# Jabruson/FDN-TIP2025

Measured on AMD Instinct MI355X. Metric: images/sec, FDN (LPNet->FDN forward) 1280x720 bs=8 fp32, higher is better.
Workload: dtype f32

## Files before the change

fdn-tip2025_amd/csrc/fft2d.hip:

```cpp
#include <math.h>

#include "common.hpp"
#include "fft_regs.hpp"

namespace {

constexpr int MAX_STAGES = FDN_FFT_MAX_STAGES;
constexpr int NT = 256;

struct Plan {
    int N;
    int nst;
    int radix[MAX_STAGES];
    const float2* tw;
    int tab_mul;
};

struct Rader {
    int p;
    const int* perm_in;
    const int* perm_out;
    const float2* bhat;
    Plan sub;
};
// ... 408 lines not shown
        float2* out2 = reinterpret_cast<float2*>(out + row0 * W);
        const int live = nrow * M;
        if (M % 2 == 0 && ((reinterpret_cast<uintptr_t>(out) | reinterpret_cast<uintptr_t>(res)) & 15) == 0) {
            const float4* res4 = reinterpret_cast<const float4*>(res2);
            float4* out4 = reinterpret_cast<float4*>(out2);
            const float4* Z4 = reinterpret_cast<const float4*>(Z);
            const int live4 = live / 2;
            for (int base = threadIdx.x; base < live4; base += NT * 4) {
                float4 r[4];
                if (res4) {
#pragma unroll
                    for (int u = 0; u < 4; ++u) r[u] = res4[min(base + NT * u, live4 - 1)];
                }
#pragma unroll
                for (int u = 0; u < 4; ++u) {
                    const int idx = base + NT * u;
                    if (idx >= live4) continue;
                    float4 v = Z4[idx];
                    v.x *= scale; v.y *= scale; v.z *= scale; v.w *= scale;
                    if (res4) {
                        v.x = fmaf(alpha, r[u].x, v.x); v.y = fmaf(alpha, r[u].y, v.y);
                        v.z = fmaf(alpha, r[u].z, v.z); v.w = fmaf(alpha, r[u].w, v.w);
                    }
                    out4[idx] = v;
                }
            }
        } else
        for (int base = threadIdx.x; base < live; base += NT * US) {
            float2 r[US];
            if (res2) {
#pragma unroll
                for (int u = 0; u < US; ++u) r[u] = res2[min(base + NT * u, live - 1)];
            }
#pragma unroll
            for (int u = 0; u < US; ++u) {
                const int idx = base + NT * u;
                if (idx >= live) continue;
                float2 v = Z[idx];
                v.x *= scale;
                v.y *= scale;
                if (res2) {
                    v.x = fmaf(alpha, r[u].x, v.x);
                    v.y = fmaf(alpha, r[u].y, v.y);
                }
                out2[idx] = v;
            }
        }
    }
}

struct ColArgs {
    float2* z;
    int H, Wf, C;
    int tc, tcs;
    long planes;
    const float4* guide;
    const float* wxa;
    const float* wxp;
    float* out_abs;
    float* out_ang;
    int rd_before;
    int fix_real;
    const float* in_mag;
    const float* in_pha;
    int Hin, Wfin;
};

enum { COL_FCAFFN = 0, COL_FWD = 1, COL_INV_POLAR = 2 };

template <int MODE, int BIG, bool INPL>
__global__ __launch_bounds__(NT, (INPL ? 2 : 1)) void fft_cols_kernel(ColArgs a, const Plan p) {
    extern __shared__ __attribute__((aligned(16))) unsigned char smem[];
    const int H = a.H, Wf = a.Wf, tc = a.tc;
    float2* A = reinterpret_cast<float2*>(smem);
    float2* Bf = A + (long)H * tc;
    float2* twl = INPL ? Bf : Bf + (long)H * tc;
    for (int i = threadIdx.x; i < H; i += NT) twl[i] = p.tw[i];
    int plane, col0;
    {
        const int ntile = (Wf + tc - 1) / tc;
        const long total = (long)ntile * a.planes, per_xcd = (total + 7) / 8;
        const long w = (long)(blockIdx.x & 7) * per_xcd + (blockIdx.x >> 3);
        if (w >= total) return;
        const int C = a.C;
        const long grp = w / C;
        const int ch = (int)(w - grp * C);
        plane = (int)(grp / ntile) * C + ch;
        col0 = (int)(grp % ntile) * tc;
    }
    const int ncol = min(tc, Wf - col0);
    float2* zp = a.z + (long)plane * H * Wf;

    const int per = H * tc, tcs = a.tcs, tcm = tc - 1;
    if (MODE == COL_INV_POLAR) {
        constexpr int U = 4;
        for (int base = threadIdx.x; base < per; base += NT * U) {
            float mg[U], ph[U];
#pragma unroll
            for (int u = 0; u < U; ++u) {
                const int idx = base + NT * u, h = idx >> tcs, c = idx & tcm;
                mg[u] = 0.f; ph[u] = 0.f;
                if (idx < per && c < ncol) {
                    const long o = ((long)plane * a.Hin + h) * a.Wfin + col0 + c;
                    mg[u] = a.in_mag[o];
                    ph[u] = a.in_pha[o];
                }
// ... 74 lines not shown
                    float sn, cs;
                    fdn_sincos(ph, &sn, &cs);
                    const float2 v = Z[idx];
                    const float2 r = make_float2(rd1(v.x), rd1(v.y));
                    Z[idx] = cmul(r, make_float2(A_ * cs, -A_ * sn));
                }
            }
        }
    }
    float2* Y = Z;
    if (INPL) fft_run_inplace<true, BIG>(Z, p, twl, tc);
    else Y = fft_run<true, BIG>(Z, other, p, twl, tc, 1, tc, true);
#pragma unroll 8
    for (int idx = threadIdx.x; idx < per; idx += NT) {
        const int h = idx >> tcs, c = idx & tcm;
        if (c < ncol) zp[(long)h * Wf + col0 + c] = Y[idx];
    }
}

using fftr::f2;
using fftr::sfor;

__device__ __forceinline__ rsrc_t cols_rsrc(const void* base, long bytes) {
    return mk_rsrc(base, (unsigned)(bytes > 0x7FFFFFFFL ? 0x7FFFFFFFL : bytes));
}

template <typename K>
int set_lds(K kernel, size_t bytes) {
    if (bytes > 48 * 1024 && !fdn_allow_dynamic_lds(reinterpret_cast<const void*>(kernel), bytes)) return FDN_ERR_LAUNCH;
    return FDN_OK;
}

template <int R, int P> struct ColPlan {
    static constexpr int NJ = R * 8, NT = NJ > 256 ? 320 : 256, KS = 256 + 4;
    static constexpr size_t lds = ((size_t)R * KS + (size_t)(P - 1) * R) * sizeof(float2);
};

template <int R, int P, int MODE>
__global__ __launch_bounds__((ColPlan<R, P>::NT), (3 * ColPlan<R, P>::lds <= 160 * 1024) ? 3 : 2) void fft_cols_rp_kernel(ColArgs a, const float2* __restrict__ twT) {
    constexpr int H = R * P, TC = 256 / P, CJ = 32 / P, NG = 8, KS = ColPlan<R, P>::KS, NJ = R * NG, NT = ColPlan<R, P>::NT;
    static_assert(TC / CJ == NG, "8 column groups");
    extern __shared__ __attribute__((aligned(16))) unsigned char smem_cols[];
    f2* Y = reinterpret_cast<f2*>(smem_cols);
    f2* twl = Y + R * KS;
    const int tid = threadIdx.x, Wf = a.Wf;
    const bool io = NT == 256 || tid < 256;
    for (int i = tid; i < (P - 1) * R; i += NT) twl[i] = f2{twT[R + i].x, twT[R + i].y};
    int plane, col0;
    {
        const int ntile = (Wf + TC - 1) / TC;
        const long total = (long)ntile * a.planes, per_xcd = (total + 7) / 8;
        const long w = (long)(blockIdx.x & 7) * per_xcd + (blockIdx.x >> 3);
        if (w >= total) return;
        const int C = a.C, CH = (C % 8 == 0) ? 8 : 1;
        const long grp = w / CH;
        const int ci = (int)(w - grp * CH);
        const long rest = grp / ntile;
        col0 = (int)(grp - rest * ntile) * TC;
        const int nchunk = C / CH;
        const long b = rest / nchunk;
        plane = (int)(b * C + (rest - b * nchunk) * CH + ci);
    }
    const int c = tid & (TC - 1), n2 = (tid & 255) / TC;
    const bool live = col0 + c < Wf;
    const int col = live ? col0 + c : Wf - 1;
    const long plane_bins = (long)H * Wf;
    const __amdgpu_buffer_rsrc_t rz = cols_rsrc(a.z + (long)plane * plane_bins, plane_bins * 8);
    const unsigned zoff = (unsigned)(n2 * Wf + col) * 8u, zstep = (unsigned)(P * Wf) * 8u;

    if (MODE != COL_INV_POLAR && io) {
        f2 u[R];
        sfor<0, R>([&](auto n1) { u[decltype(n1)::value] = bload2(rz, zoff, (unsigned)decltype(n1)::value * zstep); });
        fftr::dft_nat<R, false>(u);
        sfor<0, R>([&](auto k1) { Y[decltype(k1)::value * KS + tid] = u[decltype(k1)::value]; });
    }

    int jt = tid + 64 * (int)((blockIdx.x >> 3) % (NT / 64));
    if (jt >= NT) jt -= NT;
    const bool worker = jt < NJ;
    const int k1 = worker ? jt >> 3 : 0, cg = jt & 7;
    unsigned binq[CJ];
    bool liveq[CJ];
#pragma unroll
    for (int cc = 0; cc < CJ; ++cc) {
        liveq[cc] = col0 + cc * NG + cg < Wf;
        binq[cc] = (unsigned)(k1 * Wf + (liveq[cc] ? col0 + cc * NG + cg : Wf - 1));
    }
    const unsigned kstep = (unsigned)(R * Wf);
    constexpr int NB = (3 * ColPlan<R, P>::lds <= 160 * 1024) ? 16 : 4, BS = 32 / NB;
    fdn_u32x4 g0[2][BS];
    fdn_u32x2 g1[2][BS];
    __amdgpu_buffer_rsrc_t rg = rz;
    float wa0 = 0, wa1 = 0, wa2 = 0, wp0 = 0, wp1 = 0, wp2 = 0;
    auto gload = [&](auto bb) __attribute__((always_inline)) {
        constexpr int Bb = decltype(bb)::value;
        sfor<0, BS>([&](auto i) {
            constexpr int q = Bb * BS + decltype(i)::value, cc = q / P, k2 = fftr::brev(q % P, P);
            g0[Bb & 1][decltype(i)::value] = __builtin_amdgcn_raw_buffer_load_b128(rg, binq[cc] * 32u, (unsigned)k2 * kstep * 32u, 0);
            g1[Bb & 1][decltype(i)::value] = __builtin_amdgcn_raw_buffer_load_b64(rg, binq[cc] * 32u, (unsigned)k2 * kstep * 32u + 16u, 0);
        });
    };
    if (MODE == COL_FCAFFN) {
        const int b = plane / a.C, ch = plane - b * a.C;
        wa0 = a.wxa[ch * 3]; wa1 = a.wxa[ch * 3 + 1]; wa2 = a.wxa[ch * 3 + 2];
        wp0 = a.wxp[ch * 3]; wp1 = a.wxp[ch * 3 + 1]; wp2 = a.wxp[ch * 3 + 2];
        rg = cols_rsrc(a.guide + (long)b * plane_bins * 2, plane_bins * 32);
        if (worker) gload(std::integral_constant<int, 0>{});
// ... 88 lines not shown
            for (int cc = 0; cc < CJ; ++cc) inq[cc] = (unsigned)(k1 * a.Wfin + ((int)binq[cc] - k1 * Wf)) * 4u;
            const unsigned instep = (unsigned)(R * a.Wfin) * 4u;
            sfor<0, NB>([&](auto bb) {
                constexpr int Bb = decltype(bb)::value;
                float mg[BS], ph[BS];
                sfor<0, BS>([&](auto i) {
                    constexpr int I = decltype(i)::value, q = Bb * BS + I, cc = q / P, k2 = fftr::brev(q % P, P);
                    mg[I] = __uint_as_float(__builtin_amdgcn_raw_buffer_load_b32(rm, inq[cc], (unsigned)k2 * instep, 0));
                    ph[I] = __uint_as_float(__builtin_amdgcn_raw_buffer_load_b32(rp, inq[cc], (unsigned)k2 * instep, 0));
                });
                sfor<0, BS>([&](auto i) {
                    constexpr int I = decltype(i)::value, q = Bb * BS + I;
                    float sn, cs;
                    fdn_sincos(ph[I], &sn, &cs);
                    v[q] = f2{mg[I] * cs, mg[I] * sn};
                });
            });
        }
#pragma unroll
        for (int cc = 0; cc < CJ; ++cc) fftr::fft_dit<P, true>(v + cc * P);
        asm volatile("" ::: "memory");
        sfor<0, P>([&](auto n) {
            constexpr int N2 = decltype(n)::value;
            if constexpr (N2 > 0) {
                const f2 w = twl[(N2 - 1) * R + k1];
#pragma unroll
                for (int cc = 0; cc < CJ; ++cc) v[cc * P + N2] = fftr::cmulc(v[cc * P + N2], w);
            }
#pragma unroll
            for (int cc = 0; cc < CJ; ++cc) yb[N2 * TC + cc * NG] = v[cc * P + N2];
        });
    } else if (MODE == COL_FWD) {
        return;
    }
    __syncthreads();
    if (io) {
        f2 u[R];
        sfor<0, R>([&](auto k) { u[decltype(k)::value] = Y[decltype(k)::value * KS + tid]; });
        fftr::dft_nat<R, true>(u);
        if (live) sfor<0, R>([&](auto n1) { bstore2(u[decltype(n1)::value], rz, zoff, (unsigned)decltype(n1)::value * zstep); });
    }
}

constexpr int row_plan_groups(int R1, int P) {
    int ng = 8;
    while (ng > 1 && (R1 * ng > 256 || ((long)ng * (32 / P) * R1 * (P + 1) + (P - 1) * R1 + R1 * P + 1) * 8 > 80 * 1024)) --ng;
    return ng;
}
template <int R1, int P>
struct RowPlan {
    static constexpr int NG = row_plan_groups(R1, P);
    static constexpr int M = R1 * P, W = 2 * M, Wf = M + 1, CJ = 32 / P, RW = NG * CJ, PS = P + 1, RS = R1 * PS, NJ = R1 * NG;
    static constexpr int NTW = (P - 1) * R1 + Wf;
    static constexpr size_t lds = ((size_t)RW * RS + NTW) * sizeof(float2);
    static_assert(RW * P <= 256 && NJ <= 256 && CJ * P <= 32, "first stage: one thread per (row, n2); second stage: one per (row group, k1) with 32 values");
};

struct RowLN {
    const float* stats;
    const float* gamma;
    const float* beta;
    int C, H;
};

template <int R1, int P, bool LN = false>
__global__ __launch_bounds__(256, 2) void rfft_rows_rp_kernel(const float* __restrict__ in, float2* __restrict__ out, long R,
                                                              const float2* __restrict__ tab, RowLN lnp, int pitch) {
    typedef RowPlan<R1, P> L;
    constexpr int M = L::M, W = L::W, Wf = L::Wf, RW = L::RW, CJ = L::CJ, PS = L::PS, RS = L::RS, NJ = L::NJ;
    extern __shared__ __attribute__((aligned(16))) unsigned char smem[];
    f2* Y = reinterpret_cast<f2*>(smem);
    f2* tw2 = Y + RW * RS;
    f2* tws = tw2 + (P - 1) * R1;
    const int tid = threadIdx.x;
    for (int i = tid; i < L::NTW; i += 256) tw2[i] = f2{tab[i].x, tab[i].y};
    const long row0 = (long)blockIdx.x * RW;
    const int nrow = (int)min((long)RW, R - row0);
    {
        const int n2 = tid & (P - 1), rw = tid / P < RW ? tid / P : RW - 1;
        const int rwc = rw < nrow ? rw : nrow - 1;
        const __amdgpu_buffer_rsrc_t rin = cols_rsrc(in + row0 * W, (long)nrow * W * 4);
        const unsigned voff = (unsigned)(rwc * W + 2 * n2) * 4u;
        f2 u[R1];
        sfor<0, R1>([&](auto n1) { u[decltype(n1)::value] = bload2(rin, voff, (unsigned)(decltype(n1)::value * P * 8)); });
        if constexpr (LN) {
            const long row = row0 + rwc, plane = row / lnp.H;
            const int h = (int)(row - plane * lnp.H), c = (int)(plane % lnp.C);
            const long b = plane / lnp.C, HW = (long)lnp.H * W;
            const __amdgpu_buffer_rsrc_t rs_ = cols_rsrc(lnp.stats, (R / ((long)lnp.C * lnp.H)) * 2 * HW * 4);
            const unsigned so = (unsigned)(b * 2 * HW + h * W + 2 * n2) * 4u;
            const float ga = lnp.gamma[c], be = lnp.beta[c];
            f2 mu[R1], rs[R1];
            sfor<0, R1>([&](auto n1) {
                constexpr int N1 = decltype(n1)::value;
                mu[N1] = bload2(rs_, so, (unsigned)(N1 * P * 8));
                rs[N1] = bload2(rs_, so + (unsigned)HW * 4u, (unsigned)(N1 * P * 8));
            });
            sfor<0, R1>([&](auto n1) {
                constexpr int N1 = decltype(n1)::value;
                u[N1] = (u[N1] - mu[N1]) * rs[N1] * ga + be;
            });
        }
        fftr::dft_nat<R1, false>(u);
        sfor<0, R1>([&](auto k1) { Y[rw * RS + decltype(k1)::value * PS + n2] = u[decltype(k1)::value]; });
    }
    __syncthreads();
    const int jt = (tid + 64 * (int)(blockIdx.x & 3)) & 255;
    const bool worker = jt < NJ;
    const int rg = jt / R1, k1 = jt - rg * R1;
    f2 v[32];
    if (worker) {
        const f2* yb = Y + rg * CJ * RS + k1 * PS;
        sfor<0, P>([&](auto n) {
            constexpr int N2 = decltype(n)::value;
#pragma unroll
            for (int cc = 0; cc < CJ; ++cc) v[cc * P + N2] = yb[cc * RS + N2];
            if constexpr (N2 > 0) {
                const f2 w = tw2[(N2 - 1) * R1 + k1];
#pragma unroll
                for (int cc = 0; cc < CJ; ++cc) v[cc * P + N2] = fftr::cmul(v[cc * P + N2], w);
            }
        });
#pragma unroll
        for (int cc = 0; cc < CJ; ++cc) fftr::dft_nat<P, false>(v + cc * P);
    }
    __syncthreads();
    if (worker) {
        f2* zb = Y + rg * CJ * RS + k1;
        sfor<0, P>([&](auto k2) {
#pragma unroll
            for (int cc = 0; cc < CJ; ++cc) zb[cc * RS + R1 * decltype(k2)::value] = v[cc * P + decltype(k2)::value];
        });
    }
    __syncthreads();
    f2* out2 = reinterpret_cast<f2*>(out) + row0 * pitch;
    const int live = nrow * pitch;
    const float r_Wf = 1.0f / (float)pitch;
#pragma unroll 4
    for (int idx = tid; idx < live; idx += 256) {
        const int s = fdiv(idx, r_Wf), k = idx - s * pitch;
        if (k >= Wf) { out2[idx] = f2{0.f, 0.f}; continue; }
        const f2 zk = Y[s * RS + (k == M ? 0 : k)];
        const f2 zc = Y[s * RS + (k == 0 ? 0 : M - k)];
        const f2 e = 0.5f * f2{zk.x + zc.x, zk.y - zc.y};
        const f2 d = 0.5f * f2{zk.x - zc.x, zk.y + zc.y};
        const f2 o = fftr::mul_ni(d);
        f2 x;
        if (k == 0) x = f2{e.x + o.x, 0.0f};
        else if (k == M) x = f2{e.x - o.x, 0.0f};
        else x = e + fftr::cmul(o, tws[k]);
        out2[idx] = x;
    }
}

template <int R1, int P>
__global__ __launch_bounds__(256, 2) void irfft_rows_rp_kernel(const float2* __restrict__ in, long in_ws, long in_plane_stride,
                                                               float* __restrict__ out, int H, long R, float scale,
                                                               const float* __restrict__ res, float alpha,
                                                               const float2* __restrict__ tab) {
    typedef RowPlan<R1, P> L;
    constexpr int M = L::M, W = L::W, RW = L::RW, CJ = L::CJ, PS = L::PS, RS = L::RS, NJ = L::NJ;
    extern __shared__ __attribute__((aligned(16))) unsigned char smem[];
    f2* Y = reinterpret_cast<f2*>(smem);
    f2* tw2 = Y + RW * RS;
    f2* tws = tw2 + (P - 1) * R1;
    __shared__ long rowoff[RW];
    const int tid = threadIdx.x;
    for (int i = tid; i < L::NTW; i += 256) tw2[i] = f2{tab[i].x, tab[i].y};
    const long row0 = (long)blockIdx.x * RW;
    const int nrow = (int)min((long)RW, R - row0);
    if (tid < RW) {
        const long row = row0 + min(tid, nrow - 1);
        const long plane = row / H, h = row - plane * H;
        rowoff[tid] = plane * in_plane_stride + h * in_ws;
    }
    __syncthreads();
    {
        constexpr int UL = 4, NP = M / 2 + 1, TOT = RW * NP;
        const f2* in2 = reinterpret_cast<const f2*>(in);
        const float r_NP = 1.0f / (float)NP;
        for (int base = tid; base < TOT; base += 256 * UL) {
            f2 xks[UL], xcs[UL];
#pragma unroll
            for (int u = 0; u < UL; ++u) {
                const int idx = min(base + 256 * u, TOT - 1), s = fdiv(idx, r_NP), k = idx - s * NP;
                const f2* src = in2 + rowoff[s];
                xks[u] = src[k];
                xcs[u] = src[M - k];
            }
#pragma unroll
            for (int u = 0; u < UL; ++u) {
                const int idx = base + 256 * u;
                if (idx >= TOT) continue;
                const int s = fdiv(idx, r_NP), k = idx - s * NP;
                f2 xk = xks[u], xc = xcs[u];
                if (k == 0) { xk.y = 0.f; xc.y = 0.f; }
                const f2 e = 0.5f * f2{xk.x + xc.x, xk.y - xc.y};
                const f2 d = 0.5f * f2{xk.x - xc.x, xk.y + xc.y};
                const f2 io = fftr::mul_pi(fftr::cmulc(d, tws[k]));
                f2* row = Y + s * RS;
                row[k] = e + io;
                if (k != 0) {
                    const f2 c = e - io;
                    row[M - k] = f2{c.x, -c.y};
// ... 8 lines not shown
    f2 v[32];
    if (worker) {
        const f2* zb = Y + rg * CJ * RS + k1;
        sfor<0, P>([&](auto k2) {
#pragma unroll
            for (int cc = 0; cc < CJ; ++cc) v[cc * P + decltype(k2)::value] = zb[cc * RS + R1 * decltype(k2)::value];
        });
#pragma unroll
        for (int cc = 0; cc < CJ; ++cc) fftr::dft_nat<P, true>(v + cc * P);
    }
    __syncthreads();
    if (worker) {
        f2* yb = Y + rg * CJ * RS + k1 * PS;
        sfor<0, P>([&](auto n) {
            constexpr int N2 = decltype(n)::value;
            if constexpr (N2 > 0) {
                const f2 w = tw2[(N2 - 1) * R1 + k1];
#pragma unroll
                for (int cc = 0; cc < CJ; ++cc) v[cc * P + N2] = fftr::cmulc(v[cc * P + N2], w);
            }
#pragma unroll
            for (int cc = 0; cc < CJ; ++cc) yb[cc * RS + N2] = v[cc * P + N2];
        });
    }
    __syncthreads();
    {
        const int n2 = tid & (P - 1), rw = tid / P;
        const int rwl = rw < RW ? rw : RW - 1;
        f2 u[R1];
        sfor<0, R1>([&](auto k) { u[decltype(k)::value] = Y[rwl * RS + decltype(k)::value * PS + n2]; });
        fftr::dft_nat<R1, true>(u);
        if (rw < nrow) {
            const __amdgpu_buffer_rsrc_t ro = cols_rsrc(out + row0 * W, (long)nrow * W * 4);
            const __amdgpu_buffer_rsrc_t rr = cols_rsrc(res ? res + row0 * W : out, res ? (long)nrow * W * 4 : 0);
            const unsigned voff = (unsigned)(rw * W + 2 * n2) * 4u;
            f2 r[R1];
            if (res) sfor<0, R1>([&](auto n1) { r[decltype(n1)::value] = bload2(rr, voff, (unsigned)(decltype(n1)::value * P * 8)); });
            sfor<0, R1>([&](auto n1) {
                constexpr int N1 = decltype(n1)::value;
                f2 x = u[N1] * scale;
                if (res) x += alpha * r[N1];
                bstore2(x, ro, voff, (unsigned)(N1 * P * 8));
            });
        }
    }
}

}

#include "fft_plan.hpp"

namespace {

template <int R, int P, int MODE>
int launch_cols_rp(ColArgs a, long planes, fdn_stream_t stream) {
    const float2* tw = get_table_rp(R, P);
    if (!tw) return FDN_ERR_LAUNCH;
    a.planes = planes;
    if (a.C <= 0 || planes % a.C != 0) a.C = 1;
    constexpr int TC = 256 / P;
    const long total = (long)cdiv(a.Wf, TC) * planes, per_xcd = (total + 7) / 8;
    if (per_xcd * 8 > 0x7FFFFFFFL) return FDN_ERR_UNSUPPORTED;
    typedef ColPlan<R, P> CP;
    constexpr size_t lds = CP::lds;
    constexpr int nt = CP::NT;
    if (int e = set_lds(fft_cols_rp_kernel<R, P, MODE>, lds)) return e;
    hipLaunchKernelGGL((fft_cols_rp_kernel<R, P, MODE>), dim3((unsigned)(per_xcd * 8)), dim3(nt), lds, static_cast<hipStream_t>(stream), a, tw);
    return fdn_launch_status();
}

template <int MODE, int BIG, bool INPL>
int launch_cols_k(ColArgs a, const Plan& p, long planes, size_t lds, fdn_stream_t stream) {
    a.planes = planes;
    if (a.C <= 0 || planes % a.C != 0) a.C = 1;
    if (int e = set_lds(fft_cols_kernel<MODE, BIG, INPL>, lds)) return e;
    const long total = (long)cdiv(a.Wf, a.tc) * planes, per_xcd = (total + 7) / 8;
    if (per_xcd * 8 > 0x7FFFFFFFL) return FDN_ERR_UNSUPPORTED;
    hipLaunchKernelGGL((fft_cols_kernel<MODE, BIG, INPL>), dim3((unsigned)(per_xcd * 8)), dim3(NT), lds,
                       static_cast<hipStream_t>(stream), a, p);
    return fdn_launch_status();
}

template <int MODE>
int launch_cols(ColArgs a, long planes, fdn_stream_t stream) {
    Route r;
    cols_route(a.H, &r);
    if (r.kind == FDN_FFT_REFUSED) return FDN_ERR_UNSUPPORTED;
    if (r.kind == FDN_FFT_PLANNED)
        return col_plan(a.H, [&](auto R, auto P) { return launch_cols_rp<decltype(R)::value, decltype(P)::value, MODE>(a, planes, stream); });
    Plan p;
    if (!make_plan(a.H, a.H, &p)) return FDN_ERR_UNSUPPORTED;
    a.tc = r.width;
    a.tcs = __builtin_ctz(r.width);
    return dispatch<0, 1, 2, 4 + 0, 4 + 1>(4 * (r.kind == FDN_FFT_INPLACE) + r.big, [&](auto v) {
        constexpr int V = decltype(v)::value;
        return launch_cols_k<MODE, V % 4, V / 4 != 0>(a, p, planes, r.lds, stream);
    });
}

template <int R1, int P>
int launch_rfft_rp(const float* in, float* out_c, long rows, fdn_stream_t stream, int pitch, const RowLN* ln = nullptr) {
    typedef RowPlan<R1, P> L;
    const float2* tab = get_table_rows_rp(R1, P);
    if (!tab) return FDN_ERR_LAUNCH;
    return dispatch<0, 1>(ln != nullptr, [&](auto v) {
        constexpr bool LN = decltype(v)::value != 0;
        if (int e = set_lds(rfft_rows_rp_kernel<R1, P, LN>, L::lds)) return e;
        hipLaunchKernelGGL((rfft_rows_rp_kernel<R1, P, LN>), dim3(cdiv(rows, L::RW)), dim3(256), L::lds, static_cast<hipStream_t>(stream), in,
                           reinterpret_cast<float2*>(out_c), rows, tab, ln ? *ln : RowLN{}, pitch);
        return fdn_launch_status();
    });
}

template <int R1, int P>
int launch_irfft_rp(const float* in_c, long in_row_bins, long in_plane_bins, float* out, long planes, int H, float scale,
                    const float* res, float alpha, fdn_stream_t stream) {
    typedef RowPlan<R1, P> L;
    const float2* tab = get_table_rows_rp(R1, P);
    if (!tab) return FDN_ERR_LAUNCH;
    if (int e = set_lds(irfft_rows_rp_kernel<R1, P>, L::lds)) return e;
    const long rows = planes * H;
    hipLaunchKernelGGL((irfft_rows_rp_kernel<R1, P>), dim3(cdiv(rows, L::RW)), dim3(256), L::lds, static_cast<hipStream_t>(stream),
                       reinterpret_cast<const float2*>(in_c), in_row_bins, in_plane_bins, out, H, rows, scale, res, alpha, tab);
    return fdn_launch_status();
}

}

extern "C" int fdn_fft_prepare(int n) {
    FDN_CHECK_ARG(n > 0);
    const auto made = [](const float2* tab) { return tab ? FDN_OK : FDN_ERR_LAUNCH; };
    if (col_plan(n, [&](auto R, auto P) { return made(get_table_rp(R, P)); }) == FDN_ERR_LAUNCH) return FDN_ERR_LAUNCH;
    if (row_plan(n, [&](auto R1, auto P) { return made(get_table_rows_rp(R1, P)); }) == FDN_ERR_LAUNCH) return FDN_ERR_LAUNCH;
    return made(get_table(n));
}

extern "C" int fdn_fft_route(int kind, int n, int* desc, int ndesc) {
    FDN_CHECK_ARG(kind >= 0 && kind <= 2 && n >= 1 && desc && ndesc >= FDN_FFT_ROUTE_DESC);
    FDN_CHECK_ARG(kind == 2 || n % 2 == 0);
    for (int i = 0; i < FDN_FFT_ROUTE_DESC; ++i) desc[i] = 0;
    Route r;
    if (kind == 2) cols_route(n, &r);
    else rows_route(n, kind == 0, true, &r);
    desc[0] = r.kind;
    if (r.kind == FDN_FFT_REFUSED) return FDN_OK;
    desc[1] = r.big;
    desc[2] = r.width;
    const Plan& q = r.kind == FDN_FFT_RADER ? r.sub : r.p;
    desc[3] = r.kind == FDN_FFT_RADER ? n / 2 : 0;
    desc[4] = q.nst;
    const bool passes = r.kind == FDN_FFT_PINGPONG || r.kind == FDN_FFT_RADER;
    for (int i = 0; i < q.nst; ++i) {
        const int x = q.radix[i];
        const bool reg = x == 2 || x == 4 || x == 3 || x == 5 || x == 7 || (r.big >= 1 && (x == 17 || x == 23)) ||
                         (r.big == 2 && (x == 13 || x == 37 || x == 41));
        desc[5 + i] = x;
        desc[5 + MAX_STAGES + i] = (passes && !reg) ? 1 : 0;
    }
    return FDN_OK;
}

// ... 142 lines not shown
```

fdn-tip2025_amd/csrc/gemm_split.hip:

```cpp
#include "common.hpp"

namespace {

using f32x16 = fdn_f32x16;
typedef __bf16 bf16x8 __attribute__((ext_vector_type(8)));
__device__ __forceinline__ f32x16 mf(fdn_u32x4 a, fdn_u32x4 b, f32x16 c) {
    return __builtin_amdgcn_mfma_f32_32x32x16_bf16(__builtin_bit_cast(bf16x8, a), __builtin_bit_cast(bf16x8, b), c, 0, 0, 0);
}

constexpr int TP = 128, TN = 128, KC = 32;
constexpr int BLK = 3 * 2 * 2 * 128;
constexpr int STRIP_MAX_N = 1024;
constexpr int TRI_E = 10;

struct SArgs {
    fdn_conv1x1_desc d;
    int tiles_per_img, total_ptiles, ntiles;
    const float* xb_stats; const float* xb_gamma; const float* xb_beta;
    const float* img; const fdn_u32x4* mapw; int img_w, img_h;
};

__host__ __device__ __forceinline__ int tri_src(int kp, int E) {
    const int c = kp >> 5, hh = (kp >> 4) & 1, q = kp & 15;
    if (q == 15) return -1;
    const int j = q / 3, g = q - 3 * j, e = TRI_E * c + 5 * hh + j;
    return e < E ? g * E + e : -1;
}

template <int PRO, bool FC = false>
__global__ __launch_bounds__(256, 2) void gemm_split_kernel(SArgs a) {
    const fdn_conv1x1_desc& d = a.d;
    constexpr bool TRI = PRO == FDN_PRO_LN3_GATE, LN = PRO == FDN_PRO_LN, LNM = PRO == FDN_PRO_LN_MULADD;
    static_assert(!FC || LNM, "the FCAFFN form is the LN_MULADD prologue plus its own epilogue");
    __shared__ fdn_u32x4 Xs[BLK];
    __shared__ fdn_u32x4 Ws[BLK];
    __shared__ float red[2][TP];
    const int K = d.K, N = d.N, E = d.ln_group;
    const unsigned P = (unsigned)d.P, P4 = P * 4u;
    const int tid = threadIdx.x, lane = tid & 63, kh = lane >> 5, ln = lane & 31;
    const int wave = __builtin_amdgcn_readfirstlane(tid >> 6);
    const int wi = wave >> 1, wj = wave & 1;
    const int nch = TRI ? (E + TRI_E - 1) / TRI_E : (K + KC - 1) / KC;

    const unsigned S = xcd_contiguous(blockIdx.x, (unsigned)(a.total_ptiles * a.ntiles));
    const unsigned pt = S / (unsigned)a.ntiles;
    const int nt = (int)(S - pt * a.ntiles);
    const int b = (int)(pt / (unsigned)a.tiles_per_img);
    const unsigned p0 = (pt - (unsigned)b * a.tiles_per_img) * TP;
    const int n0 = nt * TN;

    const int xp = tid & (TP - 1), hh = wave >> 1;
    const unsigned pix = min(p0 + (unsigned)xp, P - 1);
    const int K0 = d.kseg[1] > 0 ? d.kseg[0] : K;
    const rsrc_t rx = mk_rsrc(d.x[0] + (long)b * d.xbs[0], (unsigned)K0 * P4);
    const rsrc_t rx1 = d.kseg[1] > 0 ? mk_rsrc(d.x[1] + (long)b * d.xbs[1], (unsigned)(K - K0) * P4) : rx;
    const rsrc_t rv = mk_rsrc((TRI || LNM) ? d.xb + (long)b * d.xbbs : d.x[0], TRI ? (unsigned)E * P4 : LNM ? (unsigned)K * P4 : 0u);
    const fdn_u32x4* wsrc = reinterpret_cast<const fdn_u32x4*>(d.wpk) + (long)nt * nch * BLK;
    float sa[3] = {0.f, 0.f, 0.f}, sb[3] = {0.f, 0.f, 0.f};
    if ((TRI || LN || LNM) && d.stats) {
#pragma unroll
        for (int g = 0; g < (TRI ? 3 : 1); ++g) {
            const float* sp = d.stats + ((long)b * (TRI ? 3 : 1) + g) * 2 * P;
            sa[g] = sp[P + pix];
            sb[g] = -sp[pix] * sa[g];
        }
    }
    if constexpr (TRI || LNM) {
        if (!d.stats) {
            constexpr int G = TRI ? 3 : 1;
            const int Eg = TRI ? E : K;
            float x0[G], s[G], ss[G];
#pragma unroll
            for (int g = 0; g < G; ++g) {
                x0[g] = bload(rx, pix * 4u, (unsigned)(g * Eg) * P4);
                s[g] = ss[g] = 0.f;
            }
            constexpr int PER = TRI ? 5 : 16, STEP = TRI ? TRI_E : KC;
            const int nfull = Eg / STEP;
#pragma unroll 2
            for (int c = 0; c < nfull; ++c) {
                float v[G][PER];
#pragma unroll
                for (int j = 0; j < PER; ++j)
#pragma unroll
                    for (int g = 0; g < G; ++g) v[g][j] = bload(rx, pix * 4u, (unsigned)(g * Eg + c * STEP + PER * hh + j) * P4);
#pragma unroll
                for (int j = 0; j < PER; ++j)
#pragma unroll
                    for (int g = 0; g < G; ++g) {
                        const float dl = v[g][j] - x0[g];
                        s[g] += dl;
                        ss[g] = fmaf(dl, dl, ss[g]);
                    }
            }
            for (int e = nfull * STEP + PER * hh; e < min(Eg, nfull * STEP + PER * hh + PER); ++e)
#pragma unroll
                for (int g = 0; g < G; ++g) {
                    const float dl = bload(rx, pix * 4u, (unsigned)(g * Eg + e) * P4) - x0[g];
                    s[g] += dl;
                    ss[g] = fmaf(dl, dl, ss[g]);
                }
            float* sx = reinterpret_cast<float*>(Xs);
#pragma unroll
            for (int g = 0; g < G; ++g) {
                sx[((hh * G + g) * 2 + 0) * TP + xp] = s[g];
                sx[((hh * G + g) * 2 + 1) * TP + xp] = ss[g];
            }
            __syncthreads();
            const float inv = 1.0f / (float)Eg;
#pragma unroll
            for (int g = 0; g < G; ++g) {
                const float st = sx[((0 * G + g) * 2 + 0) * TP + xp] + sx[((1 * G + g) * 2 + 0) * TP + xp];
                const float sst = sx[((0 * G + g) * 2 + 1) * TP + xp] + sx[((1 * G + g) * 2 + 1) * TP + xp];
                const float md = st * inv;
                sa[g] = 1.0f / sqrtf(fmaxf(sst * inv - md * md, 0.f) + 1e-5f);
                sb[g] = -(x0[g] + md) * sa[g];
            }
            __syncthreads();
        }
    }
    const bool x1ln = FC && a.xb_stats != nullptr;
    float sa1 = 1.f, sb1 = 0.f;
    if (x1ln) {
        const float* sp = a.xb_stats + (long)b * 2 * P;
        sa1 = sp[P + pix];
        sb1 = -sp[pix] * sa1;
    }
    float xv[16], vv[(TRI || LNM) ? (TRI ? 5 : 16) : 1];
    float ga[(TRI || LNM) ? 16 : 1], be[(TRI || LNM) ? 16 : 1];
    float g1[FC ? 16 : 1], b1[FC ? 16 : 1];
    fdn_u32x4 wv[6];
    auto fetch = [&](int c) __attribute__((always_inline)) {
        if constexpr (TRI) {
#pragma unroll
            for (int j = 0; j < 5; ++j) {
                const int e = c * TRI_E + 5 * hh + j;
                vv[j] = e < E ? bload(rv, pix * 4u, (unsigned)e * P4) : 0.f;
#pragma unroll
                for (int g = 0; g < 3; ++g) {
                    xv[3 * j + g] = e < E ? bload(rx, pix * 4u, (unsigned)(g * E + e) * P4) : 0.f;
                    ga[3 * j + g] = e < E ? d.gamma[g * E + e] : 0.f;
                    be[3 * j + g] = e < E ? d.beta[g * E + e] : 0.f;
                }
            }
        } else {
            const int k0 = c * KC + 16 * hh;
            const bool second = PRO == FDN_PRO_NONE && d.kseg[1] > 0 && k0 >= K0;
            const rsrc_t rxc = second ? rx1 : rx;
            const int kb = second ? k0 - K0 : k0;
#pragma unroll
            for (int i = 0; i < 16; ++i) {
                xv[i] = bload(rxc, pix * 4u, (unsigned)(kb + i) * P4);
                if constexpr (LNM) {
                    vv[i] = bload(rv, pix * 4u, (unsigned)(k0 + i) * P4);
                    ga[i] = k0 + i < K ? d.gamma[k0 + i] : 0.f;
                    be[i] = k0 + i < K ? d.beta[k0 + i] : 0.f;
                    if constexpr (FC) {
                        g1[i] = k0 + i < K ? (x1ln ? a.xb_gamma[k0 + i] : 1.f) : 0.f;
                        b1[i] = (x1ln && k0 + i < K) ? a.xb_beta[k0 + i] : 0.f;
                    }
                }
            }
        }
#pragma unroll
        for (int i = 0; i < 6; ++i) wv[i] = wsrc[(long)c * BLK + tid + 256 * i];
    };
    auto stash = [&](int c) __attribute__((always_inline)) {
        float v[16];
        if constexpr (TRI) {
#pragma unroll
            for (int j = 0; j < 5; ++j)
#pragma unroll
                for (int g = 0; g < 3; ++g)
                    v[3 * j + g] = fmaf(fmaf(xv[3 * j + g], sa[g], sb[g]), ga[3 * j + g], be[3 * j + g]) * vv[j];
            v[15] = 0.f;
        } else {
            const int k0 = c * KC + 16 * hh;
#pragma unroll
            for (int i = 0; i < 16; ++i) {
                if constexpr (LN) v[i] = k0 + i < K ? fmaf(xv[i], sa[0], sb[0]) : 0.f;
                else if constexpr (LNM) {
                    float x1 = vv[i];
                    if constexpr (FC) x1 = fmaf(fmaf(x1, sa1, sb1), g1[i], b1[i]);
                    v[i] = fmaf(fmaf(fmaf(xv[i], sa[0], sb[0]), ga[i], be[i]), x1, x1);
                }
                else v[i] = xv[i];
            }
        }
#pragma unroll
        for (int h = 0; h < 2; ++h) {
            fdn_u32x4 p1, p2, p3;
#pragma unroll
            for (int j = 0; j < 4; ++j) {
                const float x0 = v[8 * h + 2 * j], x1 = v[8 * h + 2 * j + 1];
                p1[j] = __builtin_amdgcn_perm(__float_as_uint(x1), __float_as_uint(x0), 0x07060302u);
                const float r0 = x0 - __uint_as_float(__float_as_uint(x0) & 0xffff0000u), r1 = x1 - __uint_as_float(__float_as_uint(x1) & 0xffff0000u);
                p2[j] = __builtin_amdgcn_perm(__float_as_uint(r1), __float_as_uint(r0), 0x07060302u);
                const float s0 = r0 - __uint_as_float(__float_as_uint(r0) & 0xffff0000u), s1 = r1 - __uint_as_float(__float_as_uint(r1) & 0xffff0000u);
                p3[j] = __builtin_amdgcn_perm(__float_as_uint(s1), __float_as_uint(s0), 0x07060302u);
            }
            Xs[((0 * 2 + hh) * 2 + h) * 128 + xp] = p1;
            Xs[((1 * 2 + hh) * 2 + h) * 128 + xp] = p2;
            Xs[((2 * 2 + hh) * 2 + h) * 128 + xp] = p3;
        }
#pragma unroll
        for (int i = 0; i < 6; ++i) Ws[tid + 256 * i] = wv[i];
    };

    f32x16 acc[2][2];
#pragma unroll
    for (int s = 0; s < 2; ++s)
#pragma unroll
        for (int t = 0; t < 2; ++t)
#pragma unroll
            for (int r = 0; r < 16; ++r) acc[s][t][r] = 0.f;

    fetch(0);
    stash(0);
    __syncthreads();
    const fdn_u32x4* xb_ = Xs + kh * 128 + wi * 64 + ln;
    const fdn_u32x4* wb_ = Ws + kh * 128 + wj * 64 + ln;
    for (int c = 0; c < nch; ++c) {
        const bool more = c + 1 < nch;
        if (more) fetch(c + 1);
#pragma unroll
        for (int ks = 0; ks < 2; ++ks) {
            fdn_u32x4 A[2][3], B[2][3];
#pragma unroll
            for (int p = 0; p < 3; ++p)
#pragma unroll
                for (int s = 0; s < 2; ++s) {
                    B[s][p] = xb_[((p * 2 + ks) * 2) * 128 + s * 32];
                    A[s][p] = wb_[((p * 2 + ks) * 2) * 128 + s * 32];
                }
#pragma unroll
            for (int s = 0; s < 2; ++s)
#pragma unroll
                for (int t = 0; t < 2; ++t) {
                    acc[s][t] = mf(A[t][2], B[s][0], acc[s][t]);
                    acc[s][t] = mf(A[t][1], B[s][1], acc[s][t]);
                    acc[s][t] = mf(A[t][0], B[s][2], acc[s][t]);
                    acc[s][t] = mf(A[t][1], B[s][0], acc[s][t]);
                    acc[s][t] = mf(A[t][0], B[s][1], acc[s][t]);
                    acc[s][t] = mf(A[t][0], B[s][0], acc[s][t]);
                }
        }
        __syncthreads();
        if (more) stash(c + 1);
        __syncthreads();
    }

    const int Nt = min(N - n0, TN);
    const rsrc_t ro = mk_rsrc(d.out + (long)b * d.obs + (long)n0 * P, (unsigned)Nt * P4);
    const bool RES = d.epi == FDN_EPI_RES, MA = d.epi == FDN_EPI_MULADD;
    const rsrc_t rr = mk_rsrc(RES ? d.res + (long)b * d.rbs + (long)n0 * P : MA ? d.mul + (long)b * d.mbs + (long)n0 * P : d.out, (RES || MA) ? (unsigned)Nt * P4 : 0u);
    const rsrc_t ra = mk_rsrc(MA ? d.add + (long)b * d.mbs + (long)n0 * P : d.out, MA ? (unsigned)Nt * P4 : 0u);
    const rsrc_t rbias = mk_rsrc(d.bias ? d.bias + n0 : d.w, d.bias ? (unsigned)Nt * 4u : 0u);
    if constexpr (FC) {
        const int Wd = a.img_w, Hh = a.img_h;
        const rsrc_t ri = mk_rsrc(a.img + (long)b * 3 * P, 3u * P4);
        fdn_u32x4 Bm[2][2][3];
#pragma unroll
        for (int s = 0; s < 2; ++s) {
            const unsigned pc = min(p0 + (unsigned)(wi * 64 + s * 32 + ln), P - 1);
            const int y = (int)(pc / (unsigned)Wd), x = (int)pc - y * Wd;
            const bool up = y > 0, dn = y < Hh - 1, lf = x > 0, rt = x < Wd - 1;
#pragma unroll
            for (int ks = 0; ks < 2; ++ks) {
                float v[8];
#pragma unroll
                for (int j = 0; j < 8; ++j) {
                    const int kk0 = 16 * ks + j, kk1 = kk0 + 8;
                    const int t0 = kk0 / 3, c0 = kk0 - 3 * t0, dy0 = t0 / 3 - 1, dx0 = t0 % 3 - 1;
                    const int t1 = kk1 / 3, c1 = kk1 - 3 * t1, dy1 = t1 / 3 - 1, dx1 = t1 % 3 - 1;
                    const bool in0 = kk0 < 27 && (dy0 < 0 ? up : dy0 > 0 ? dn : true) && (dx0 < 0 ? lf : dx0 > 0 ? rt : true);
                    const bool in1 = kk1 < 27 && (dy1 < 0 ? up : dy1 > 0 ? dn : true) && (dx1 < 0 ? lf : dx1 > 0 ? rt : true);
                    const int off0 = c0 * (int)P + dy0 * Wd + dx0, off1 = c1 * (int)P + dy1 * Wd + dx1;
                    const bool in = kh ? in1 : in0;
                    const int off = kh ? off1 : off0;
                    v[j] = bload(ri, in ? (unsigned)((int)pc + off) * 4u : 0x80000000u, 0u);
                }
#pragma unroll
                for (int j = 0; j < 4; ++j) {
                    unsigned u1, u2, u3;
                    fdn_split3(v[2 * j], v[2 * j + 1], u1, u2, u3);
                    Bm[s][ks][0][j] = u1; Bm[s][ks][1][j] = u2; Bm[s][ks][2][j] = u3;
                }
            }
        }
        const int nt32 = (N + 31) / 32;
        const rsrc_t rb = mk_rsrc(d.bias ? d.bias + n0 : d.w, d.bias ? (unsigned)min(N - n0, TN) * 4u : 0u);
#pragma unroll
        for (int m = 0; m < 2; ++m) {
            f32x16 mac[2][2];
#pragma unroll
            for (int s = 0; s < 2; ++s)
#pragma unroll
                for (int t = 0; t < 2; ++t)
#pragma unroll
                    for (int r = 0; r < 16; ++r) mac[s][t][r] = 0.f;
#pragma unroll
            for (int ks = 0; ks < 2; ++ks)
// ... 480 lines not shown
```

Before: 28.29.

## Reuse LN stats across channels in row FFT and keep GEMM inputs in registers

The row rFFT kernel with fused layer-norm now gives each block a group of channels for the same batch and row range. It loads the per-pixel mean and rstd once and loops over the channels, prefetching the next channel's input while it runs the current FFT. In the split GEMM, when K is small and stats are computed in-kernel, the activation values read for the statistics pass are kept in registers and reused for staging, so they are not fetched from global memory twice. The column kernel's channel chunk also becomes a host parameter, now set to C. The cost is more register pressure, extra syncs per channel iteration, and fewer blocks in the row grid.

```diff
diff --git a/fdn-tip2025_amd/csrc/fft2d.hip b/fdn-tip2025_amd/csrc/fft2d.hip
--- a/fdn-tip2025_amd/csrc/fft2d.hip
+++ b/fdn-tip2025_amd/csrc/fft2d.hip
@@ -484,6 +484,7 @@
 struct ColArgs {
     float2* z;
     int H, Wf, C;
+    int ch;
     int tc, tcs;
     long planes;
     const float4* guide;
@@ -664,7 +665,7 @@
         const long total = (long)ntile * a.planes, per_xcd = (total + 7) / 8;
         const long w = (long)(blockIdx.x & 7) * per_xcd + (blockIdx.x >> 3);
         if (w >= total) return;
-        const int C = a.C, CH = (C % 8 == 0) ? 8 : 1;
+        const int C = a.C, CH = a.ch;
         const long grp = w / CH;
         const int ci = (int)(w - grp * CH);
         const long rest = grp / ntile;
@@ -859,6 +860,7 @@
     static constexpr int NG = row_plan_groups(R1, P);
     static constexpr int M = R1 * P, W = 2 * M, Wf = M + 1, CJ = 32 / P, RW = NG * CJ, PS = P + 1, RS = R1 * PS, NJ = R1 * NG;
     static constexpr int NTW = (P - 1) * R1 + Wf;
+    static constexpr int CG = R1 != 20 ? 1 : P == 32 ? 8 : P == 16 ? 4 : 2;
     static constexpr size_t lds = ((size_t)RW * RS + NTW) * sizeof(float2);
     static_assert(RW * P <= 256 && NJ <= 256 && CJ * P <= 32, "first stage: one thread per (row, n2); second stage: one per (row group, k1) with 32 values");
 };
@@ -874,89 +876,116 @@
 __global__ __launch_bounds__(256, 2) void rfft_rows_rp_kernel(const float* __restrict__ in, float2* __restrict__ out, long R,
                                                               const float2* __restrict__ tab, RowLN lnp, int pitch) {
     typedef RowPlan<R1, P> L;
-    constexpr int M = L::M, W = L::W, Wf = L::Wf, RW = L::RW, CJ = L::CJ, PS = L::PS, RS = L::RS, NJ = L::NJ;
+    constexpr int M = L::M, W = L::W, Wf = L::Wf, RW = L::RW, CJ = L::CJ, PS = L::PS, RS = L::RS, NJ = L::NJ, CG = LN ? L::CG : 1;
     extern __shared__ __attribute__((aligned(16))) unsigned char smem[];
     f2* Y = reinterpret_cast<f2*>(smem);
     f2* tw2 = Y + RW * RS;
     f2* tws = tw2 + (P - 1) * R1;
     const int tid = threadIdx.x;
     for (int i = tid; i < L::NTW; i += 256) tw2[i] = f2{tab[i].x, tab[i].y};
-    const long row0 = (long)blockIdx.x * RW;
-    const int nrow = (int)min((long)RW, R - row0);
-    {
-        const int n2 = tid & (P - 1), rw = tid / P < RW ? tid / P : RW - 1;
-        const int rwc = rw < nrow ? rw : nrow - 1;
-        const __amdgpu_buffer_rsrc_t rin = cols_rsrc(in + row0 * W, (long)nrow * W * 4);
-        const unsigned voff = (unsigned)(rwc * W + 2 * n2) * 4u;
-        f2 u[R1];
+    long row0 = (long)blockIdx.x * RW;
+    int nrow, nch = 1, c0 = 0, h0 = 0, b = 0;
+    if constexpr (LN) {
+        const unsigned nrg = (unsigned)(lnp.H + RW - 1) / RW, ncg = (unsigned)(lnp.C + CG - 1) / CG;
+        const unsigned S = xcd_contiguous(blockIdx.x, gridDim.x);
+        const unsigned t = S / ncg, cgi = S - t * ncg;
+        b = (int)(t / nrg);
+        h0 = (int)(t - (unsigned)b * nrg) * RW;
+        c0 = (int)cgi * CG;
+        nch = min(CG, lnp.C - c0);
+        nrow = min(RW, lnp.H - h0);
+        row0 = ((long)b * lnp.C + c0) * lnp.H + h0;
+    } else {
+        nrow = (int)min((long)RW, R - row0);
+    }
+    const int n2 = tid & (P - 1), rw = tid / P < RW ? tid / P : RW - 1;
+    const int rwc = rw < nrow ? rw : nrow - 1;
+    const unsigned voff = (unsigned)(rwc * W + 2 * n2) * 4u;
+    const long pstep = LN ? (long)lnp.H : 0;
+    auto xload = [&](int j, f2* u) __attribute__((always_inline)) {
+        const __amdgpu_buffer_rsrc_t rin = cols_rsrc(in + (row0 + (long)min(j, nch - 1) * pstep) * W, j < nch ? (long)nrow * W * 4 : 0);
         sfor<0, R1>([&](auto n1) { u[decltype(n1)::value] = bload2(rin, voff, (unsigned)(decltype(n1)::value * P * 8)); });
-        if constexpr (LN) {
-            const long row = row0 + rwc, plane = row / lnp.H;
-            const int h = (int)(row - plane * lnp.H), c = (int)(plane % lnp.C);
-            const long b = plane / lnp.C, HW = (long)lnp.H * W;
-            const __amdgpu_buffer_rsrc_t rs_ = cols_rsrc(lnp.stats, (R / ((long)lnp.C * lnp.H)) * 2 * HW * 4);
-            const unsigned so = (unsigned)(b * 2 * HW + h * W + 2 * n2) * 4u;
-            const float ga = lnp.gamma[c], be = lnp.beta[c];
-            f2 mu[R1], rs[R1];
-            sfor<0, R1>([&](auto n1) {
-                constexpr int N1 = decltype(n1)::value;
-                mu[N1] = bload2(rs_, so, (unsigned)(N1 * P * 8));
-                rs[N1] = bload2(rs_, so + (unsigned)HW * 4u, (unsigned)(N1 * P * 8));
-            });
-            sfor<0, R1>([&](auto n1) {
-                constexpr int N1 = decltype(n1)::value;
-                u[N1] = (u[N1] - mu[N1]) * rs[N1] * ga + be;
-            });
-        }
-        fftr::dft_nat<R1, false>(u);
-        sfor<0, R1>([&](auto k1) { Y[rw * RS + decltype(k1)::value * PS + n2] = u[decltype(k1)::value]; });
-    }
-    __syncthreads();
+    };
+    f2 mu[LN ? R1 : 1], rs[LN ? R1 : 1];
+    auto normalise = [&](int j, f2* u) __attribute__((always_inline)) {
+        const int c = c0 + min(j, nch - 1);
+        const float ga = lnp.gamma[c], be = lnp.beta[c];
+        sfor<0, R1>([&](auto n1) {
+            constexpr int N1 = decltype(n1)::value;
+            u[N1] = (u[N1] - mu[N1]) * rs[N1] * ga + be;
+        });
+    };
+    f2 u[R1];
+    xload(0, u);
+    if constexpr (LN) {
+        const long HW = (long)lnp.H * W;
+        const __amdgpu_buffer_rsrc_t rs_ = cols_rsrc(lnp.stats + (long)b * 2 * HW, 2 * HW * 4);
+        const unsigned so = (unsigned)((h0 + rwc) * W + 2 * n2) * 4u;
+        sfor<0, R1>([&](auto n1) {
+            constexpr int N1 = decltype(n1)::value;
+            mu[N1] = bload2(rs_, so, (unsigned)(N1 * P * 8));
+            rs[N1] = bload2(rs_, so + (unsigned)HW * 4u, (unsigned)(N1 * P * 8));
+        });
+        normalise(0, u);
+    }
     const int jt = (tid + 64 * (int)(blockIdx.x & 3)) & 255;
     const bool worker = jt < NJ;
     const int rg = jt / R1, k1 = jt - rg * R1;
-    f2 v[32];
-    if (worker) {
-        const f2* yb = Y + rg * CJ * RS + k1 * PS;
-        sfor<0, P>([&](auto n) {
-            constexpr int N2 = decltype(n)::value;
-#pragma unroll
-            for (int cc = 0; cc < CJ; ++cc) v[cc * P + N2] = yb[cc * RS + N2];
-            if constexpr (N2 > 0) {
-                const f2 w = tw2[(N2 - 1) * R1 + k1];
-#pragma unroll
-                for (int cc = 0; cc < CJ; ++cc) v[cc * P + N2] = fftr::cmul(v[cc * P + N2], w);
-            }
-        });
-#pragma unroll
-        for (int cc = 0; cc < CJ; ++cc) fftr::dft_nat<P, false>(v + cc * P);
-    }
-    __syncthreads();
-    if (worker) {
-        f2* zb = Y + rg * CJ * RS + k1;
-        sfor<0, P>([&](auto k2) {
-#pragma unroll
-            for (int cc = 0; cc < CJ; ++cc) zb[cc * RS + R1 * decltype(k2)::value] = v[cc * P + decltype(k2)::value];
-        });
-    }
-    __syncthreads();
-    f2* out2 = reinterpret_cast<f2*>(out) + row0 * pitch;
+    const float r_Wf = 1.0f / (float)pitch;
     const int live = nrow * pitch;
-    const float r_Wf = 1.0f / (float)pitch;
+#pragma unroll 1
+    for (int j = 0; j < nch; ++j) {
+        f2 un[CG > 1 ? R1 : 1];
+        if constexpr (CG > 1) xload(j + 1, un);
+        fftr::dft_nat<R1, false>(u);
+        sfor<0, R1>([&](auto k1_) { Y[rw * RS + decltype(k1_)::value * PS + n2] = u[decltype(k1_)::value]; });
+        __syncthreads();
+        f2 v[32];
+        if (worker) {
+            const f2* yb = Y + rg * CJ * RS + k1 * PS;
+            sfor<0, P>([&](auto n) {
+                constexpr int N2 = decltype(n)::value;
+#pragma unroll
+                for (int cc = 0; cc < CJ; ++cc) v[cc * P + N2] = yb[cc * RS + N2];
+                if constexpr (N2 > 0) {
+                    const f2 w = tw2[(N2 - 1) * R1 + k1];
+#pragma unroll
+                    for (int cc = 0; cc < CJ; ++cc) v[cc * P + N2] = fftr::cmul(v[cc * P + N2], w);
+                }
+            });
+#pragma unroll
+            for (int cc = 0; cc < CJ; ++cc) fftr::dft_nat<P, false>(v + cc * P);
+        }
+        __syncthreads();
+        if (worker) {
+            f2* zb = Y + rg * CJ * RS + k1;
+            sfor<0, P>([&](auto k2) {
+#pragma unroll
+                for (int cc = 0; cc < CJ; ++cc) zb[cc * RS + R1 * decltype(k2)::value] = v[cc * P + decltype(k2)::value];
+            });
+        }
+        __syncthreads();
+        if constexpr (CG > 1) {
+            sfor<0, R1>([&](auto n1) { u[decltype(n1)::value] = un[decltype(n1)::value]; });
+            normalise(j + 1, u);
+        }
+        f2* out2 = reinterpret_cast<f2*>(out) + (row0 + (long)j * pstep) * pitch;
 #pragma unroll 4
-    for (int idx = tid; idx < live; idx += 256) {
-        const int s = fdiv(idx, r_Wf), k = idx - s * pitch;
-        if (k >= Wf) { out2[idx] = f2{0.f, 0.f}; continue; }
-        const f2 zk = Y[s * RS + (k == M ? 0 : k)];
-        const f2 zc = Y[s * RS + (k == 0 ? 0 : M - k)];
-        const f2 e = 0.5f * f2{zk.x + zc.x, zk.y - zc.y};
-        const f2 d = 0.5f * f2{zk.x - zc.x, zk.y + zc.y};
-        const f2 o = fftr::mul_ni(d);
-        f2 x;
-        if (k == 0) x = f2{e.x + o.x, 0.0f};
-        else if (k == M) x = f2{e.x - o.x, 0.0f};
-        else x = e + fftr::cmul(o, tws[k]);
-        out2[idx] = x;
+        for (int idx = tid; idx < live; idx += 256) {
+            const int s = fdiv(idx, r_Wf), k = idx - s * pitch;
+            if (k >= Wf) { out2[idx] = f2{0.f, 0.f}; continue; }
+            const f2 zk = Y[s * RS + (k == M ? 0 : k)];
+            const f2 zc = Y[s * RS + (k == 0 ? 0 : M - k)];
+            const f2 e = 0.5f * f2{zk.x + zc.x, zk.y - zc.y};
+            const f2 d = 0.5f * f2{zk.x - zc.x, zk.y + zc.y};
+            const f2 o = fftr::mul_ni(d);
+            f2 x;
+            if (k == 0) x = f2{e.x + o.x, 0.0f};
+            else if (k == M) x = f2{e.x - o.x, 0.0f};
+            else x = e + fftr::cmul(o, tws[k]);
+            out2[idx] = x;
+        }
+        if constexpr (CG > 1) __syncthreads();
     }
 }
 
@@ -1071,12 +1100,15 @@
 
 namespace {
 
+int cols_chunk(int C) { return C; }
+
 template <int R, int P, int MODE>
 int launch_cols_rp(ColArgs a, long planes, fdn_stream_t stream) {
     const float2* tw = get_table_rp(R, P);
     if (!tw) return FDN_ERR_LAUNCH;
     a.planes = planes;
     if (a.C <= 0 || planes % a.C != 0) a.C = 1;
+    a.ch = cols_chunk(a.C);
     constexpr int TC = 256 / P;
     const long total = (long)cdiv(a.Wf, TC) * planes, per_xcd = (total + 7) / 8;
     if (per_xcd * 8 > 0x7FFFFFFFL) return FDN_ERR_UNSUPPORTED;
@@ -1122,10 +1154,12 @@
     typedef RowPlan<R1, P> L;
     const float2* tab = get_table_rows_rp(R1, P);
     if (!tab) return FDN_ERR_LAUNCH;
-    return dispatch<0, 1>(ln != nullptr, [&](auto v) {
+    return dispatch<0, 1>(ln != nullptr, [&](auto v) -> int {
         constexpr bool LN = decltype(v)::value != 0;
         if (int e = set_lds(rfft_rows_rp_kernel<R1, P, LN>, L::lds)) return e;
-        hipLaunchKernelGGL((rfft_rows_rp_kernel<R1, P, LN>), dim3(cdiv(rows, L::RW)), dim3(256), L::lds, static_cast<hipStream_t>(stream), in,
+        const long items = ln ? rows / ln->H / ln->C * cdiv(ln->H, L::RW) * cdiv(ln->C, L::CG) : cdiv(rows, L::RW);
+        if (items > 0x7FFFFFFFL) return FDN_ERR_UNSUPPORTED;
+        hipLaunchKernelGGL((rfft_rows_rp_kernel<R1, P, LN>), dim3((unsigned)items), dim3(256), L::lds, static_cast<hipStream_t>(stream), in,
                            reinterpret_cast<float2*>(out_c), rows, tab, ln ? *ln : RowLN{}, pitch);
         return fdn_launch_status();
     });
diff --git a/fdn-tip2025_amd/csrc/gemm_split.hip b/fdn-tip2025_amd/csrc/gemm_split.hip
--- a/fdn-tip2025_amd/csrc/gemm_split.hip
+++ b/fdn-tip2025_amd/csrc/gemm_split.hip
@@ -57,6 +57,9 @@
     const rsrc_t rv = mk_rsrc((TRI || LNM) ? d.xb + (long)b * d.xbbs : d.x[0], TRI ? (unsigned)E * P4 : LNM ? (unsigned)K * P4 : 0u);
     const fdn_u32x4* wsrc = reinterpret_cast<const fdn_u32x4*>(d.wpk) + (long)nt * nch * BLK;
     float sa[3] = {0.f, 0.f, 0.f}, sb[3] = {0.f, 0.f, 0.f};
+    constexpr int KEEP = 4;
+    float xk[FC ? KEEP : 1][16];
+    const bool keep = FC && !d.stats && K <= KEEP * KC;
     if ((TRI || LN || LNM) && d.stats) {
 #pragma unroll
         for (int g = 0; g < (TRI ? 3 : 1); ++g) {
@@ -76,7 +79,24 @@
                 s[g] = ss[g] = 0.f;
             }
             constexpr int PER = TRI ? 5 : 16, STEP = TRI ? TRI_E : KC;
-            const int nfull = Eg / STEP;
+            const int nfull = keep ? 0 : Eg / STEP;
+            if constexpr (FC) {
+                if (keep) {
+#pragma unroll
+                    for (int c = 0; c < KEEP; ++c)
+#pragma unroll
+                        for (int j = 0; j < 16; ++j) xk[c][j] = bload(rx, pix * 4u, (unsigned)(c * KC + 16 * hh + j) * P4);
+#pragma unroll
+                    for (int c = 0; c < KEEP; ++c)
+#pragma unroll
+                        for (int j = 0; j < 16; ++j)
+                            if (c * KC + 16 * hh + j < K) {
+                                const float dl = xk[c][j] - x0[0];
+                                s[0] += dl;
+                                ss[0] = fmaf(dl, dl, ss[0]);
+                            }
+                }
+            }
 #pragma unroll 2
             for (int c = 0; c < nfull; ++c) {
                 float v[G][PER];
@@ -93,7 +113,7 @@
                         ss[g] = fmaf(dl, dl, ss[g]);
                     }
             }
-            for (int e = nfull * STEP + PER * hh; e < min(Eg, nfull * STEP + PER * hh + PER); ++e)
+            for (int e = nfull * STEP + PER * hh; !keep && e < min(Eg, nfull * STEP + PER * hh + PER); ++e)
 #pragma unroll
                 for (int g = 0; g < G; ++g) {
                     const float dl = bload(rx, pix * 4u, (unsigned)(g * Eg + e) * P4) - x0[g];
@@ -130,7 +150,7 @@
     float ga[(TRI || LNM) ? 16 : 1], be[(TRI || LNM) ? 16 : 1];
     float g1[FC ? 16 : 1], b1[FC ? 16 : 1];
     fdn_u32x4 wv[6];
-    auto fetch = [&](int c) __attribute__((always_inline)) {
+    auto fetch = [&](int c, auto with_x) __attribute__((always_inline)) {
         if constexpr (TRI) {
 #pragma unroll
             for (int j = 0; j < 5; ++j) {
@@ -150,7 +170,7 @@
             const int kb = second ? k0 - K0 : k0;
 #pragma unroll
             for (int i = 0; i < 16; ++i) {
-                xv[i] = bload(rxc, pix * 4u, (unsigned)(kb + i) * P4);
+                if constexpr (decltype(with_x)::value) xv[i] = bload(rxc, pix * 4u, (unsigned)(kb + i) * P4);
                 if constexpr (LNM) {
                     vv[i] = bload(rv, pix * 4u, (unsigned)(k0 + i) * P4);
                     ga[i] = k0 + i < K ? d.gamma[k0 + i] : 0.f;
@@ -165,7 +185,7 @@
 #pragma unroll
         for (int i = 0; i < 6; ++i) wv[i] = wsrc[(long)c * BLK + tid + 256 * i];
     };
-    auto stash = [&](int c) __attribute__((always_inline)) {
+    auto stash = [&](int c, const float* xv) __attribute__((always_inline)) {
         float v[16];
         if constexpr (TRI) {
 #pragma unroll
@@ -215,14 +235,9 @@
 #pragma unroll
             for (int r = 0; r < 16; ++r) acc[s][t][r] = 0.f;
 
-    fetch(0);
-    stash(0);
-    __syncthreads();
     const fdn_u32x4* xb_ = Xs + kh * 128 + wi * 64 + ln;
     const fdn_u32x4* wb_ = Ws + kh * 128 + wj * 64 + ln;
-    for (int c = 0; c < nch; ++c) {
-        const bool more = c + 1 < nch;
-        if (more) fetch(c + 1);
+    auto product = [&]() __attribute__((always_inline)) {
 #pragma unroll
         for (int ks = 0; ks < 2; ++ks) {
             fdn_u32x4 A[2][3], B[2][3];
@@ -245,9 +260,37 @@
                     acc[s][t] = mf(A[t][0], B[s][0], acc[s][t]);
                 }
         }
+    };
+    if constexpr (FC) {
+        if (keep) {
+            fetch(0, std::false_type{});
+            stash(0, xk[0]);
+            __syncthreads();
+#pragma unroll
+            for (int c = 0; c < KEEP; ++c) {
+                if (c < nch) {
+                    const bool more = c + 1 < nch;
+                    if (more) fetch(c + 1, std::false_type{});
+                    product();
+                    __syncthreads();
+                    if (more) stash(c + 1, xk[c + 1 < KEEP ? c + 1 : KEEP - 1]);
+                    __syncthreads();
+                }
+            }
+        }
+    }
+    if (!keep) {
+        fetch(0, std::true_type{});
+        stash(0, xv);
         __syncthreads();
-        if (more) stash(c + 1);
-        __syncthreads();
+        for (int c = 0; c < nch; ++c) {
+            const bool more = c + 1 < nch;
+            if (more) fetch(c + 1, std::true_type{});
+            product();
+            __syncthreads();
+            if (more) stash(c + 1, xv);
+            __syncthreads();
+        }
     }
 
     const int Nt = min(N - n0, TN);
```

New measurement: 28.20. Within noise of the previous version (-0.3%).
